# nikkolasg/playsnark

Measured on AMD Instinct MI355X. Metric: G1 scalar-muls/s (Pippenger MSM, 2^20 pts per GPU), higher is better.
Workload: dtype i32x14 (381-bit Fp, 28-bit unsaturated limbs, Montgomery); 1 GPU; BLS12-381 G1 MSM, 2^20 points per GPU, uniform 255-bit scalars; points_per_gpu=1048576, window_bits=20, windows=13, window_table=True, window_table_bytes=1744830464, slice=32, in_flight=4

## Files before the change

playsnark_amd/csrc/capi.hip:

```cpp
#include "../../include/playsnark_hip.h"

#include <hip/hip_runtime.h>

#include <algorithm>
#include <atomic>
#include <chrono>
#include <condition_variable>
#include <functional>
#include <mutex>
#include <cstdio>
#include <cstring>
#include <future>
#include <string>
#include <vector>

#include "msm.hpp"
#include "quotient.hpp"
#include "lagrange.hpp"

namespace ps {
#include "hostfield.inc"
}
using namespace ps;

// ... 970 lines not shown
                           (u32*)c->offs.p);
        hipLaunchKernelGGL(k_sort_big_scatter, dim3(big_grid), dim3(SORT_FINE), 0, st, (const unsigned short*)c->keys.p,
                           (const u32*)c->vals.p, (const u32*)coarse_off, (const u32*)tile_base, ncoarse, fb, (u32*)c->counts.p,
                           (u32*)c->sorted.p);
        }
    } else {
        HIP_TRY(hipMemsetAsync(c->counts.p, 0, 4 * G, st));
        {
            int bin_shift = 4;
            while ((pl.NB >> bin_shift) > (u32)DIGITS_BINS) bin_shift++;
            hipLaunchKernelGGL(k_digits_grouped, dgrid, dim3(DIGITS_THREADS), 2 * DIGITS_CHUNK * sizeof(u32), st, scalars_ptr(sc),
                               (u32)n, pl.c, pl.W, pl.NB, cadd, bin_shift, fold_neg, single, (u32*)c->counts.p, (u32*)c->keys.p,
                               (u32*)c->vals.p, (u32*)c->ranks.p);
        }
        PS_STAGE_MARK();
        hipLaunchKernelGGL(k_scan_blocks, dim3(scan_tiles), dim3(SCAN_BLOCK), 0, st, (const u32*)c->counts.p, (u32*)c->offs.p,
                           (u32*)c->bsum.p, (u64)G);
        hipLaunchKernelGGL(k_scan_top, dim3(1), dim3(1024), 0, st, (u32*)c->bsum.p, scan_tiles, (u32*)c->offs.p + G);
        hipLaunchKernelGGL(k_scan_add, dim3(scan_tiles), dim3(SCAN_BLOCK), 0, st, (u32*)c->offs.p, (const u32*)c->bsum.p, (u64)G);
        PS_STAGE_MARK();
        hipLaunchKernelGGL(k_scatter, dim3(nblocks(total)), dim3(256), 0, st, (const u32*)c->keys.p, (const u32*)c->vals.p,
                           (const u32*)c->ranks.p, (const u32*)c->offs.p, total, (u32*)c->sorted.p);
    }
    PS_STAGE_MARK();
    HIP_TRY(hipGetLastError());
    if (!pl.qtail) HIP_TRY(hipMemcpyAsync((char*)c->h_pinned + c->h_pinned_cap - 8, (u32*)c->offs.p + G, 4, hipMemcpyDeviceToHost, st));
    return PS_OK;
}

struct TableRef { const char* base; u64 stride; };
static bool table_ref(const ps_points* pts, size_t n, int wbits, int W, TableRef* out) {
    const Storage* st = pts->st;
    const size_t rb = table_row_bytes(pts->group);
    if (const void* t = st->table.load(std::memory_order_acquire)) {
        if (st->table_c == wbits && W <= st->table_W) {
            *out = TableRef{(const char*)t + pts->first * rb, (u64)st->table_stride};
            return true;
        }
    }
    if (const ViewTable* v = view_table_find(st, pts->first, n, wbits)) {
        const void* t = v->table.load(std::memory_order_acquire);
        if (t && W <= v->W) {
            *out = TableRef{(const char*)t, (u64)v->n};
            return true;
        }
    }
    return false;
}

template <class F>
static int msm_points_t(ps_ctx* c, ps_ctx* wc, const ps_points* pts, size_t n, const MsmPlan& pl, bool timed, int slot,
                        hipEvent_t wait_acc, hipEvent_t acc_done, bool inline_tail = false) {
    typedef typename KernelField<F>::type KF;
    constexpr unsigned LN = FieldTraits<KF>::LANES;
    const u64 total = (u64)pl.W * n;
    const u64 G = pl.G;
    const u32 nthreads_acc = (u32)((total + pl.M - 1) / pl.M);
    ReducePlan rp = reduce_plan(pl.NB);
    if (pl.qtail) {
        rp.small = false;
        rp.njobs = (u32)pl.c;
        rp.nblk = 1;
        rp.m = 0;
        rp.segs = ((1u << (pl.c - 1 - pl.rc_s)) + (1u << pl.rc_s) + 1) / 2;
    }
    const u32 nseg_total = rp.segs * (u32)pl.sets;
    const u32 per_role = rp.m * (u32)pl.sets, nres = rp.njobs * (u32)pl.sets;
    const bool tab = pl.table;
    const u32 pstride = tab ? (u32)table_row_bytes(pts->group) : (u32)sizeof(Affine<F>);
    TableRef tref{};
    if (tab && !table_ref(pts, n, pl.c, pl.W, &tref)) return fail(PS_ERR_ARG, "msm: internal: the plan names a window table the array does not carry");
    const char* src = tab ? tref.base : (const char*)points_ptr(pts);
    const u32 idx_mask = tab ? (1u << ENTRY_W_SHIFT) - 1u : 0x7fffffffu;
    const u64 w_stride = tab ? tref.stride : 0ull;
    int rc;
    if ((rc = wc->buckets.ensure(sizeof(Xyzz<F>) * G))) return rc;
    if ((rc = wc->parts.ensure(sizeof(Xyzz<F>) * 2 * (size_t)nthreads_acc))) return rc;
    if ((rc = wc->segs.ensure(sizeof(Xyzz<F>) * (2 * (size_t)nseg_total + 5 * (size_t)per_role + (size_t)nres * rp.nblk)))) return rc;
    if ((rc = wc->wins.ensure(sizeof(Xyzz<F>) * ((size_t)nres + (size_t)pl.sets) + 16))) return rc;
    const bool qfix = pl.shortsum && pl.lpb >= 1;
    const u32 qlpb = qfix ? std::min<u32>((u32)pl.lpb, 256 / QTraits<KF>::GL) : 0;
    const u64 heavy_slices = qfix ? std::min<u64>(HEAVY_SPAN, (u64)QFIX_HEAVY * qlpb - 1) : HEAVY_SPAN;
    const size_t max_heavy = (size_t)(total / (heavy_slices * (u64)pl.M)) + 2;
    if ((rc = wc->heavy.ensure(4 * (2 * max_heavy + 2)))) return rc;
    const u32 heavy_npb = 256 / QTraits<KF>::GL;
    const size_t max_jobs = (size_t)nthreads_acc / heavy_npb + max_heavy + 1;
    if ((rc = wc->hparts.ensure(sizeof(Xyzz<F>) * max_jobs))) return rc;
    if (sizeof(Xyzz<F>) * (pl.sets > 1 ? (size_t)pl.sets : (size_t)nres) + 16 > PS_PINNED_SLOT) return fail(PS_ERR_ARG, "too many windows");
    hipStream_t st = wc->stream;
    int evi = 4;
    if (wc->tail_used) HIP_TRY(hipStreamWaitEvent(st, wc->ev_tail_done, 0));
    if (storage_wait_ready(pts->st, st)) return fail(PS_ERR_HIP, "msm: event wait failed");
    if (wait_acc) HIP_TRY(hipStreamWaitEvent(st, wait_acc, 0));
    PS_STAGE_MARK();
    constexpr bool PF = LN == 1 || PS_G2_ACC_WAVES == 1;
    hipLaunchKernelGGL((k_accumulate<KF, PF>), dim3(nblocks((size_t)nthreads_acc * LN)), dim3(256), 0, st, src,
                       (const u32*)c->sorted.p, (const u32*)c->offs.p, (u32)G, pl.M, nthreads_acc, idx_mask, w_stride, pstride,
                       (Xyzz<F>*)wc->buckets.p, (Xyzz<F>*)wc->parts.p, (u32*)wc->heavy.p);
    if (acc_done) HIP_TRY(hipEventRecord(acc_done, st));
    PS_STAGE_MARK();
    HIP_TRY(hipEventRecord(wc->ev_acc_local, st));
    if (!inline_tail) {
        st = wc->tail;
        HIP_TRY(hipStreamWaitEvent(st, wc->ev_acc_local, 0));
    }
    if (pl.shortsum && pl.lpb >= 1) {
        const u32 lpb = qlpb;
        hipLaunchKernelGGL(k_qfixup<KF>, dim3(nblocks(G * (u64)lpb * QTraits<KF>::GL)), dim3(256), 0, st, (const u32*)c->offs.p, (u32)G, pl.M,
                           nthreads_acc, lpb, (const Xyzz<F>*)wc->parts.p, (Xyzz<F>*)wc->buckets.p, (u32*)wc->heavy.p, (u32*)wc->heavy.p + 1);
    } else
    hipLaunchKernelGGL(k_fixup<KF>, dim3(nblocks(G * LN)), dim3(256), 0, st, (const u32*)c->offs.p, (u32)G, pl.M, nthreads_acc,
                       (const Xyzz<F>*)wc->parts.p, (Xyzz<F>*)wc->buckets.p, (u32*)wc->heavy.p, (u32*)wc->heavy.p + 1);
    {
        const u32* hcount = (const u32*)wc->heavy.p;
        const u32* hlist = hcount + 1;
        u32* job_base = (u32*)wc->heavy.p + 1 + max_heavy;
        hipLaunchKernelGGL(k_heavy_jobs, dim3(1), dim3(256), 0, st, (const u32*)c->offs.p, (u32)G, pl.M, nthreads_acc, hcount, hlist, job_base, heavy_npb);
        hipLaunchKernelGGL(k_qfixup_heavy_part<KF>, dim3(1024), dim3(256), 0, st, (const u32*)c->offs.p, (u32)G, pl.M, nthreads_acc,
                           (const Xyzz<F>*)wc->parts.p,
                           hcount, hlist, (const u32*)job_base, (Xyzz<F>*)wc->hparts.p);
        hipLaunchKernelGGL(k_qfixup_heavy<KF>, dim3(256), dim3(256), 0, st, (const Xyzz<F>*)wc->hparts.p, (Xyzz<F>*)wc->buckets.p, hcount,
                           hlist, (const u32*)job_base);
    }
    PS_STAGE_MARK();
    {
        Xyzz<F>* accs = (Xyzz<F>*)wc->segs.p;
        Xyzz<F>* runs = accs + nseg_total;
        Xyzz<F>* lvl = runs + nseg_total;
        Xyzz<F>* pieces = lvl + 5 * (size_t)per_role;
        if (pl.qtail) {
            constexpr u32 QGL = QTraits<KF>::GL, QNP = 512 / QGL;
            const int cb = pl.c - 1, s = pl.rc_s;
            const u32 rows = 1u << (cb - s), cols = 1u << s;
            Xyzz<F>* R = accs;
            Xyzz<F>* C = accs + (size_t)pl.sets * rows;
            if (s > 0) {
                u32 np = std::min<u32>(QNP, std::max(rows, cols));
                while (np > 64 / QGL && (u64)np * QGL * (rows + cols) * (u32)pl.sets > 2048ull * 64) np >>= 1;
#if defined(PS_TAIL_TUNE)
                if (pl.busy) if (const char* e = getenv("PS_T_NP_BUSY")) np = std::max<u32>(64 / QGL, std::min<u32>(np, (u32)atoi(e)));
#endif
                hipLaunchKernelGGL(k_qreduce_rowcol<KF>, dim3((rows + cols) * (u32)pl.sets), dim3(np * QGL), np * QGL * sizeof(Fp), st,
                                   (const Xyzz<F>*)wc->buckets.p, cb, s, R, C, (const Xyzz<F>*)nullptr, (Xyzz<F>*)nullptr);
            }
            const u32 terms = std::max(rows, cols / 2);
            const u32 np = std::min<u32>(QNP, std::max<u32>(terms, 64 / QGL));
            hipLaunchKernelGGL(k_qreduce_bits<KF>, dim3(nres), dim3(np * QGL), np * QGL * sizeof(Fp), st,
                               s > 0 ? (const Xyzz<F>*)R : (const Xyzz<F>*)wc->buckets.p, (const Xyzz<F>*)C, cb, s, (Xyzz<F>*)wc->wins.p,
                               (const u32*)c->offs.p + G, (u32*)((Xyzz<F>*)wc->wins.p + (pl.sets > 1 ? nres + (size_t)pl.sets : (size_t)nres)),
                               (const Xyzz<F>*)nullptr);
        } else if (rp.small) {
            hipLaunchKernelGGL(k_reduce_small<KF>, dim3(nres), dim3(RED_SUM_LANES * LN), RED_SUM_LANES * sizeof(Xyzz<F>), st,
                               (const Xyzz<F>*)wc->buckets.p, pl.NB, rp.njobs, (Xyzz<F>*)wc->wins.p);
        } else {
            hipLaunchKernelGGL(k_reduce_l1<KF>, dim3(nblocks((size_t)nseg_total * LN)), dim3(256), 0, st, (const Xyzz<F>*)wc->buckets.p,
                               nseg_total, accs, runs);
            if (pl.hybrid && rp.segs >= 64) {
                constexpr u32 QGL = QTraits<KF>::GL, QNP = 256 / QGL;
                int cb2 = 0;
                while ((1u << cb2) < rp.segs) cb2++;
                const int s2 = (cb2 + 1) / 2;
                const u32 rows2 = 1u << (cb2 - s2), cols2 = 1u << s2;
                Xyzz<F>* R_run = lvl;
                Xyzz<F>* C_run = R_run + (size_t)pl.sets * rows2;
                Xyzz<F>* R_acc = C_run + (size_t)pl.sets * cols2;
                u32 np = std::min<u32>(QNP, std::max(rows2, cols2));
                while (np > 64 / QGL && (u64)np * QGL * (2 * rows2 + cols2) * (u32)pl.sets > 2048ull * 64) np >>= 1;
                hipLaunchKernelGGL(k_qreduce_rowcol<KF>, dim3((2 * rows2 + cols2) * (u32)pl.sets), dim3(np * QGL), np * QGL * sizeof(Fp), st,
                                   (const Xyzz<F>*)runs, cb2, s2, R_run, C_run, (const Xyzz<F>*)accs, R_acc);
                const u32 np2 = std::min<u32>(QNP, std::max<u32>(std::max(rows2, cols2 / 2), 64 / QGL));
                hipLaunchKernelGGL(k_qreduce_bits<KF>, dim3(nres), dim3(np2 * QGL), np2 * QGL * sizeof(Fp), st, (const Xyzz<F>*)R_run,
                                   (const Xyzz<F>*)C_run, cb2, s2, (Xyzz<F>*)wc->wins.p, (const u32*)nullptr, (u32*)nullptr, (const Xyzz<F>*)R_acc);
            } else {
            hipLaunchKernelGGL(k_reduce_pyr<KF>, dim3(nblocks(5 * (size_t)per_role * LN)), dim3(256), 0, st, (const Xyzz<F>*)accs,
                               (const Xyzz<F>*)runs, rp.segs, rp.m, (u32)pl.sets, lvl);
            hipLaunchKernelGGL(k_reduce_sum<KF>, dim3(nres * rp.nblk), dim3(RED_SUM_LANES * LN), RED_SUM_LANES * sizeof(Xyzz<F>), st,
                               (const Xyzz<F>*)lvl, rp.m, (u32)pl.sets, rp.njobs, rp.nblk, rp.nblk > 1 ? pieces : (Xyzz<F>*)wc->wins.p);
            if (rp.nblk > 1)
                hipLaunchKernelGGL(k_reduce_fin<KF>, dim3(nres), dim3(RED_SUM_LANES * LN), RED_SUM_LANES * sizeof(Xyzz<F>), st,
                                   (const Xyzz<F>*)pieces, rp.nblk, (Xyzz<F>*)wc->wins.p);
            }
        }
        if (pl.sets > 1)
            hipLaunchKernelGGL(k_reduce_weights<KF>, dim3((unsigned)pl.sets), dim3(RED_SUM_LANES * LN), RED_SUM_LANES * sizeof(Xyzz<F>), st,
                               (const Xyzz<F>*)wc->wins.p, rp.njobs, (rp.small && !pl.qtail) ? 1 : 0, pl.qtail ? 0 : RED_SEG_LOG,
                               (Xyzz<F>*)wc->wins.p + nres);
    }
    PS_STAGE_MARK();
    HIP_TRY(hipGetLastError());
    HIP_TRY(hipMemcpyAsync((char*)c->h_pinned + (size_t)slot * PS_PINNED_SLOT, (const Xyzz<F>*)wc->wins.p + (pl.sets > 1 ? nres : 0),
                           sizeof(Xyzz<F>) * (pl.sets > 1 ? (size_t)pl.sets : (size_t)nres) + (pl.qtail ? 4 : 0), hipMemcpyDeviceToHost, st));
    HIP_TRY(hipEventRecord(wc->ev_tail_done, st));
    wc->tail_used = true;
    return PS_OK;
}
#undef PS_STAGE_MARK

static bool table_usable(const ps_ctx* c, const ps_points* pts, size_t n, int max_bits) {
    const Storage* st = pts->st;
// ... 575 lines not shown
```

playsnark_amd/csrc/msm.hpp:

```cpp
#pragma once
#include "curve.hpp"

namespace ps {

#ifndef PS_TAIL_PRIO
#define PS_TAIL_PRIO 0
#endif
#if PS_TAIL_PRIO > 0
#define PS_TAIL_PRIO_HERE __builtin_amdgcn_s_setprio(PS_TAIL_PRIO)
#else
#define PS_TAIL_PRIO_HERE do { } while (0)
#endif

struct MsmPlan {
    int c;
    int W;
    u32 NB;
    u64 G;
    int M;
    int SEG;
    int sets;
    bool table;
    bool qtail;
    bool hybrid;
    bool shortsum;
    int lpb;
    int rc_s;
    bool busy;
};
constexpr int ENTRY_W_SHIFT = 26;

static inline MsmPlan msm_plan(size_t n, int max_bits, int forced_c) {
    MsmPlan best{};
    double best_cost = 1e300;
    for (int c = 4; c <= 20; c++) {
        if (forced_c ? c != forced_c : c > 16) continue;
        int W = max_bits / c + 1;
        double nb = (double)(1u << (c - 1));
        double cost = (double)n * W * 10.0 + W * nb * 42.0;
        if (cost < best_cost) {
            best_cost = cost;
            best.c = c;
            best.W = W;
        }
    }
    best.NB = 1u << (best.c - 1);
    best.sets = best.W;
    best.G = (u64)best.W * best.NB;
    best.M = 32;
    const u64 total = (u64)n * best.W;
    while (best.M < 1024 && total / (2 * (u64)best.M) >= (1u << 19)) best.M *= 2;
    while (best.M < 1024 && (u64)best.M * 5 * best.G < total) best.M *= 2;
    while (best.M > 8 && total / (u64)best.M < (1u << 17) && (u64)(best.M / 2) * 5 * best.G >= total) best.M /= 2;
    best.SEG = 8;
    return best;
}
static inline MsmPlan msm_plan_table(size_t n, int max_bits, int c) {
    MsmPlan pl{};
    pl.c = c;
    pl.W = max_bits / c + 1;
    pl.NB = 1u << (c - 1);
    pl.sets = 1;
    pl.table = true;
    pl.G = pl.NB;
    pl.M = 32;
    const u64 total = (u64)n * pl.W;
    while (pl.M < 1024 && total / (2 * (u64)pl.M) >= (1u << 19)) pl.M *= 2;
    while (pl.M < 1024 && (u64)pl.M * 5 * pl.G < total) pl.M *= 2;
    while (pl.M > 8 && total / (u64)pl.M < (1u << 17) && (u64)(pl.M / 2) * 5 * pl.G >= total) pl.M /= 2;
    pl.SEG = 8;
    return pl;
}

PS_INL u32 limb_sel8(const u32* k, int i) {
    u32 v = 0;
#pragma unroll
    for (int j = 0; j < 8; j++) v = (i == j) ? k[j] : v;
    return v;
}
constexpr int DIGITS_THREADS = 1024;
#ifndef PS_DIGITS_PER_THREAD
#define PS_DIGITS_PER_THREAD 8
#endif
constexpr int DIGITS_PER_THREAD = PS_DIGITS_PER_THREAD;
// ... 522 lines not shown
    __shared__ u32 hist[SORT_FINE];
    const u32 tid = threadIdx.x;
    for (u32 t = blockIdx.x;; t += gridDim.x) {
        u32 p, lo, hi;
        if (!sort_big_tile(t, tile_base, coarse_off, ncoarse, &p, &lo, &hi)) return;
        hist[tid] = 0;
        __syncthreads();
        u32 k[SORT_TILE_PER_THREAD];
#pragma unroll
        for (u32 j = 0; j < SORT_TILE_PER_THREAD; j++) {
            const u32 i = lo + j * SORT_FINE + tid;
            const bool act = i < hi;
            k[j] = act ? (u32)part_key[i] : 0xffffffffu;
            lds_count(hist, act ? k[j] : 0u, act);
        }
        __syncthreads();
        const u32 cnt = hist[tid];
        __syncthreads();
        hist[tid] = (tid < (1u << fb) && cnt) ? atomicAdd(&gcur[((size_t)p << fb) + tid], cnt) : 0u;
        __syncthreads();
#pragma unroll
        for (u32 j = 0; j < SORT_TILE_PER_THREAD; j++) {
            const bool act = k[j] != 0xffffffffu;
            const u32 pos = lds_rank(hist, act ? k[j] : 0u, act);
            if (act) sorted[pos] = part_val[lo + j * SORT_FINE + tid];
        }
        __syncthreads();
    }
}

template <class KF> struct FieldTraits { typedef KF Store; static constexpr int LANES = 1; };
template <> struct FieldTraits<Fp2s> { typedef Fp2 Store; static constexpr int LANES = 2; };
template <class S> struct KernelField { typedef S type; };
template <> struct KernelField<Fp2> { typedef Fp2s type; };

__device__ inline Fp ld_f(const Fp* p, const Fp*) { return *p; }
__device__ inline void st_f(Fp* p, const Fp& v) { *p = v; }
__device__ inline Fp2s ld_f(const Fp2* p, const Fp2s*) { return Fp2s{pair_lane() ? p->c1 : p->c0}; }
__device__ inline void st_f(Fp2* p, const Fp2s& v) { if (pair_lane()) p->c1 = v.v; else p->c0 = v.v; }

template <class KF>
__device__ inline Affine<KF> ld_affine(const Affine<typename FieldTraits<KF>::Store>* p) {
    Affine<KF> r;
    r.x = ld_f(&p->x, (const KF*)0);
    r.y = ld_f(&p->y, (const KF*)0);
    return r;
}
template <class KF>
__device__ inline Xyzz<KF> ld_xyzz(const Xyzz<typename FieldTraits<KF>::Store>* p) {
    Xyzz<KF> r;
    r.x = ld_f(&p->x, (const KF*)0);
    r.y = ld_f(&p->y, (const KF*)0);
    r.zz = ld_f(&p->zz, (const KF*)0);
    r.zzz = ld_f(&p->zzz, (const KF*)0);
    return r;
}
template <class KF>
__device__ inline void st_xyzz(Xyzz<typename FieldTraits<KF>::Store>* p, const Xyzz<KF>& v) {
    st_f(&p->x, v.x);
    st_f(&p->y, v.y);
    st_f(&p->zz, v.zz);
    st_f(&p->zzz, v.zzz);
}
template <class KF> __device__ inline u32 logical_tid() { return (blockIdx.x * blockDim.x + threadIdx.x) / FieldTraits<KF>::LANES; }
template <class KF> __device__ inline u32 logical_local() { return threadIdx.x / FieldTraits<KF>::LANES; }
template <class KF> __device__ inline u32 logical_block() { return blockDim.x / FieldTraits<KF>::LANES; }
template <class KF> __device__ inline bool pair_leader() { return FieldTraits<KF>::LANES == 1 || pair_lane() == 0; }

template <class KF>
__device__ inline void block_tree_sum(Xyzz<typename FieldTraits<KF>::Store>* sm, const Xyzz<KF>& mine) {
    const u32 lt = logical_local<KF>();
    st_xyzz<KF>(&sm[lt], mine);
    __syncthreads();
    for (u32 stride = logical_block<KF>() >> 1; stride > 0; stride >>= 1) {
        if (lt < stride) {
            Xyzz<KF> a = ld_xyzz<KF>(&sm[lt]), b = ld_xyzz<KF>(&sm[lt + stride]);
            xyzz_add_inl<KF>(a, b);
            st_xyzz<KF>(&sm[lt], a);
        }
        __syncthreads();
    }
}

__device__ inline int eff_slice(u32 E, u32 T, int M) {
#if defined(PS_NO_EFF_SLICE)
    return M;
#endif
    const u64 m = (4ull * E + T - 1) / (T ? T : 1u);
    const u64 lo = M < 4 ? (u64)M : 4ull;
    return m >= (u64)M ? M : (int)(m < lo ? lo : m);
}

template <class F>
PS_INL bool affine_is_identity(const Affine<F>& p) { return fp_all_zero(p.x) && fp_all_zero(p.y); }

template <class KF>
__device__ inline void flush_run(const Xyzz<KF>& acc, u32 g, u32 rs, u32 re, u32 slice_start, u32 t,
                                 const u32* __restrict__ offs, Xyzz<typename FieldTraits<KF>::Store>* __restrict__ buckets,
                                 Xyzz<typename FieldTraits<KF>::Store>* __restrict__ parts) {
    bool whole = (rs == offs[g]) && (re == offs[g + 1]);
    if (whole) st_xyzz<KF>(&buckets[g], acc);
    else if (rs == slice_start) st_xyzz<KF>(&parts[2 * (size_t)t], acc);
    else st_xyzz<KF>(&parts[2 * (size_t)t + 1], acc);
}

template <class KF>
__device__ inline Affine<KF> ld_entry_point(const char* __restrict__ points, u32 e, u32 idx_mask, u64 w_stride, u32 pstride) {
    const size_t row = (size_t)(e & idx_mask) + (size_t)((e >> ENTRY_W_SHIFT) & 31u) * w_stride;
    return ld_affine<KF>(reinterpret_cast<const Affine<typename FieldTraits<KF>::Store>*>(points + row * pstride));
}

__device__ inline void next_bucket(const u32* __restrict__ offs, u32 G, u32 p, u32& g, u32& bend) {
    g++;
    bend = offs[g + 1];
    if (bend > p) return;
    u32 lo = g + 1, hi = G;
    while (hi - lo > 1) {
        const u32 mid = (lo + hi) >> 1;
        if (offs[mid] <= p) lo = mid; else hi = mid;
    }
    g = lo;
    bend = offs[g + 1];
}

#ifndef PS_G2_ACC_WAVES
#define PS_G2_ACC_WAVES 2
#endif
#define PS_ACC_WAVES(KF) (FieldTraits<KF>::LANES == 2 ? PS_G2_ACC_WAVES : 2)
template <class KF, bool PREFETCH>
__global__ void __launch_bounds__(256, PS_ACC_WAVES(KF)) k_accumulate(const char* __restrict__ points,
                                                       const u32* __restrict__ sorted, const u32* __restrict__ offs,
                                                       u32 G, int Mplan, u32 T, u32 idx_mask, u64 w_stride, u32 pstride,
                                                       Xyzz<typename FieldTraits<KF>::Store>* __restrict__ buckets,
                                                       Xyzz<typename FieldTraits<KF>::Store>* __restrict__ parts,
                                                       u32* __restrict__ heavy_count) {
    const u32 E = offs[G];
    const int M = eff_slice(E, T, Mplan);
    const u32 t = logical_tid<KF>();
    if (blockIdx.x == 0 && threadIdx.x == 0) *heavy_count = 0;
    const u64 start64 = (u64)t * (u64)M;
    if (start64 >= E) return;
    const u32 start = (u32)start64;
    const u32 end = (E - start < (u32)M) ? E : start + (u32)M;
    u32 lo = 0, hi = G;
    while (hi - lo > 1) {
        u32 mid = (lo + hi) >> 1;
        if (offs[mid] <= start) lo = mid; else hi = mid;
    }
    u32 g = lo;
    u32 bend = offs[g + 1];
    u32 run_start = start;
    Xyzz<KF> acc = xyzz_identity<KF>();
    if (PREFETCH) {
        u32 e = sorted[start];
        u32 e1 = start + 1 < end ? sorted[start + 1] : e;
        Affine<KF> pt = ld_entry_point<KF>(points, e, idx_mask, w_stride, pstride);
        for (u32 p = start; p < end; p++) {
            Affine<KF> nxt = pt;
            u32 e2 = e1;
            if (p + 1 < end) nxt = ld_entry_point<KF>(points, e1, idx_mask, w_stride, pstride);
            if (p + 2 < end) e2 = sorted[p + 2];
            if (p >= bend) {
                flush_run<KF>(acc, g, run_start, p, start, t, offs, buckets, parts);
                acc = xyzz_identity<KF>();
                run_start = p;
                next_bucket(offs, G, p, g, bend);
            }
            if (!affine_is_identity<KF>(pt)) {
                if (e >> 31) pt.y = f_neg(pt.y);
                xyzz_madd_inl<KF>(acc, pt.x, pt.y);
            }
            pt = nxt; e = e1; e1 = e2;
        }
    } else {
        for (u32 p = start; p < end; p++) {
            if (p >= bend) {
                flush_run<KF>(acc, g, run_start, p, start, t, offs, buckets, parts);
                acc = xyzz_identity<KF>();
                run_start = p;
                next_bucket(offs, G, p, g, bend);
            }
            const u32 e = sorted[p];
            Affine<KF> pt = ld_entry_point<KF>(points, e, idx_mask, w_stride, pstride);
            if (!affine_is_identity<KF>(pt)) {
                if (e >> 31) pt.y = f_neg(pt.y);
                xyzz_madd_inl<KF>(acc, pt.x, pt.y);
            }
        }
    }
    flush_run<KF>(acc, g, run_start, end, start, t, offs, buckets, parts);
}

constexpr u32 HEAVY_SPAN = 8;

#ifndef PS_TAIL_WAVES
#define PS_TAIL_WAVES 2
#endif

template <class KF>
__global__ void __launch_bounds__(256, PS_TAIL_WAVES) k_fixup(const u32* __restrict__ offs, u32 G, int Mplan, u32 T,
                                                  const Xyzz<typename FieldTraits<KF>::Store>* __restrict__ parts,
                                                  Xyzz<typename FieldTraits<KF>::Store>* __restrict__ buckets,
                                                  u32* __restrict__ heavy_count, u32* __restrict__ heavy_list) {
    PS_TAIL_PRIO_HERE;
    u32 g = logical_tid<KF>();
    if (g >= G) return;
    const int M = eff_slice(offs[G], T, Mplan);
    u32 lo = offs[g], hi = offs[g + 1];
    if (lo == hi) {
        st_xyzz<KF>(&buckets[g], xyzz_identity<KF>());
        return;
    }
    u32 t0 = lo / (u32)M, t1 = (hi - 1) / (u32)M;
    if (t0 == t1) return;
    if (t1 - t0 >= HEAVY_SPAN) {
        if (pair_leader<KF>()) heavy_list[atomicAdd(heavy_count, 1u)] = g;
        return;
    }
    Xyzz<KF> acc = xyzz_identity<KF>();
    for (u32 t = t0; t <= t1; t++) {
        u32 slice_start = t * (u32)M;
        u32 rs = lo > slice_start ? lo : slice_start;
        Xyzz<KF> part = ld_xyzz<KF>(&parts[2 * (size_t)t + (rs == slice_start ? 0 : 1)]);
        xyzz_add_inl<KF>(acc, part);
    }
    st_xyzz<KF>(&buckets[g], acc);
}

constexpr u32 HEAVY_CHUNK = 1024;
__host__ __device__ inline u32 heavy_chunk_of(u32 span, u32 npb) {
    u32 s = 1;
    while ((u64)s * s * npb * npb < span) s++;
    return npb * s;
}

__global__ void __launch_bounds__(256) k_heavy_jobs(const u32* __restrict__ offs, u32 G, int Mplan, u32 T, const u32* __restrict__ heavy_count,
                                                    const u32* __restrict__ heavy_list, u32* __restrict__ job_base, u32 npb) {
    PS_TAIL_PRIO_HERE;
    const int M = eff_slice(offs[G], T, Mplan);
    __shared__ u32 wsum[4];
    const u32 nheavy = *heavy_count;
    const u32 tid = threadIdx.x;
    u32 running = 0;
    for (u32 base = 0; base < nheavy; base += 256) {
        const u32 h = base + tid;
        u32 cnt = 0;
        if (h < nheavy) {
            const u32 g = heavy_list[h];
            const u32 t0 = offs[g] / (u32)M, t1 = (offs[g + 1] - 1) / (u32)M;
            const u32 chunk = npb ? heavy_chunk_of(t1 - t0 + 1, npb) : HEAVY_CHUNK;
            cnt = (t1 - t0 + chunk) / chunk;
        }
        u32 inc = wave_incl_scan(cnt);
        if ((tid & 63) == 63) wsum[tid >> 6] = inc;
        __syncthreads();
        u32 before = 0, tile = 0;
        for (u32 q = 0; q < 4; q++) {
            if (q < (tid >> 6)) before += wsum[q];
            tile += wsum[q];
        }
        if (h < nheavy) job_base[h] = running + before + inc - cnt;
        running += tile;
        __syncthreads();
    }
    if (tid == 0) job_base[nheavy] = running;
}


#ifndef PS_RED_SEG_LOG
#define PS_RED_SEG_LOG 3
#endif
constexpr int RED_SEG_LOG = PS_RED_SEG_LOG;
constexpr int RED_SEG = 1 << RED_SEG_LOG;
constexpr int RED_DIRECT_JOBS = 4;
constexpr u32 RED_SUM_LANES = 64;
#ifndef PS_RED_SUM_TERMS
#define PS_RED_SUM_TERMS 512
#endif
constexpr u32 RED_SUM_TERMS = PS_RED_SUM_TERMS;

struct ReducePlan {
    u32 segs;
    u32 m;
    int kb;
    u32 njobs;
    u32 nblk;
    bool small;
};
constexpr u32 RED_SMALL_NB = 1024;
static inline ReducePlan reduce_plan(u32 NB) {
    ReducePlan r;
    r.small = NB <= RED_SMALL_NB;
    if (r.small) {
        r.segs = r.m = 0;
        r.kb = 0;
        r.njobs = 1;
        while ((1u << (r.njobs - 1)) < NB) r.njobs++;
        r.nblk = 1;
        return r;
    }
    r.segs = NB >> RED_SEG_LOG;
    r.m = r.segs >= 8 ? r.segs / 8 : 1;
    r.kb = 0;
    while ((1u << r.kb) < r.m) r.kb++;
    r.njobs = RED_DIRECT_JOBS + (u32)r.kb;
    r.nblk = r.m / RED_SUM_TERMS;
    if (r.nblk < 1) r.nblk = 1;
    if (r.nblk > RED_SUM_LANES) r.nblk = RED_SUM_LANES;
// ... 469 lines not shown
```

playsnark_amd/csrc/qtail.hpp:

```cpp
#pragma once

namespace ps {

template <class KF> struct QTraits {
    static constexpr int S = FieldTraits<KF>::LANES;
    static constexpr int GL = 4 * S;
};
PS_INL Fp& fp_of(Fp& a) { return a; }
PS_INL const Fp& fp_of(const Fp& a) { return a; }
PS_INL Fp& fp_of(Fp2s& a) { return a.v; }
PS_INL const Fp& fp_of(const Fp2s& a) { return a.v; }

#if defined(__HIP_DEVICE_COMPILE__)
__device__ inline i32 lane_read(i32 v, int src_lane) { return __builtin_amdgcn_ds_bpermute(src_lane << 2, v); }
#else
PS_HD inline i32 lane_read(i32 v, int) { return v; }
#endif

template <class KF> __device__ inline int q_coord() { return (int)((threadIdx.x / QTraits<KF>::S) & 3u); }

template <class KF>
__device__ inline KF q_get(const KF& v, int src) {
    constexpr int S = QTraits<KF>::S;
    const int lane = (int)(threadIdx.x & 63u);
// ... 80 lines not shown
        fp_of(ob).l[i] = odd ? fp_of(b).l[i] : fp_of(d).l[i];
    }
    const KF e = f_mul_ilp(oa, ob);
    const KF PP = q_bcast<0>(e), Pd = q_bcast<1>(d);
#pragma unroll
    for (int i = 0; i < FP_L; i++) {
        fp_of(oa).l[i] = j == 0 ? fp_of(m).l[i] : j == 1 ? fp_of(e).l[i] : fp_of(Pd).l[i];
        fp_of(ob).l[i] = j == 0 ? fp_of(e).l[i] : fp_of(PP).l[i];
    }
    const KF f = f_mul_ilp(oa, ob);
    const KF QQ = q_bcast<0>(f);
    const KF x3 = f_norm(f_sub(f_sub(f_sub(e, f), QQ), QQ));
    const KF x3q = f_sub(x3, QQ);
    KF oc, od;
#pragma unroll
    for (int i = 0; i < FP_L; i++) {
        fp_of(oa).l[i] = j == 2 ? fp_of(d).l[i] : fp_of(e).l[i];
        fp_of(ob).l[i] = j == 2 ? fp_of(x3q).l[i] : fp_of(f).l[i];
        fp_of(oc).l[i] = j == 2 ? fp_of(m).l[i] : 0;
        fp_of(od).l[i] = j == 2 ? fp_of(f).l[i] : 0;
    }
    const KF g = f_mul2sub_ilp(oa, ob, oc, od);
    const KF X3 = q_bcast<2>(x3);
    a = q_select<KF>(X3, f, f_norm(g), g, j);
}

template <class KF>
__device__ inline void q_block_tree(Fp* sm, KF& mine, u32 pt, u32 grp) {
    constexpr u32 GL = QTraits<KF>::GL;
    const u32 sub = pt & (grp - 1);
    for (u32 stride = grp >> 1; stride > 0; stride >>= 1) {
        if (sub >= stride && sub < 2 * stride) sm[threadIdx.x] = fp_of(mine);
        __syncthreads();
        if (sub < stride) {
            KF o;
            fp_of(o) = sm[threadIdx.x + stride * GL];
            q_add<KF>(mine, o);
        }
    }
}

constexpr u32 QFIX_HEAVY = 16;
template <class KF>
__global__ void __launch_bounds__(256) k_qfixup(const u32* __restrict__ offs, u32 G, int Mplan, u32 T, u32 LPB,
                                                const Xyzz<typename FieldTraits<KF>::Store>* __restrict__ parts,
                                                Xyzz<typename FieldTraits<KF>::Store>* __restrict__ buckets,
                                                u32* __restrict__ heavy_count, u32* __restrict__ heavy_list) {
    PS_TAIL_PRIO_HERE;
    constexpr u32 GL = QTraits<KF>::GL;
    __shared__ Fp sm[256];
    const int M = eff_slice(offs[G], T, Mplan);
    const u32 pt = threadIdx.x / GL;
    const u64 gp = (u64)blockIdx.x * (256 / GL) + pt;
    const u32 g = (u32)(gp / LPB), sub = (u32)(gp % LPB);
    const bool valid = g < G;
    KF acc = f_zero((const KF*)0);
    bool store = false;
    if (valid) {
        const u32 lo = offs[g], hi = offs[g + 1];
        if (lo == hi) {
            store = true;
        } else {
            const u32 t0 = lo / (u32)M, t1 = (hi - 1) / (u32)M;
            if (t0 != t1) {
                if (t1 - t0 >= QFIX_HEAVY * LPB) {
                    if (sub == 0 && (threadIdx.x & (GL - 1)) == 0) heavy_list[atomicAdd(heavy_count, 1u)] = g;
                } else {
                    store = true;
                    for (u32 t = t0 + sub; t <= t1; t += LPB) {
                        const u32 slice_start = t * (u32)M;
                        const u32 rs = lo > slice_start ? lo : slice_start;
                        const KF p = q_load<KF>(&parts[2 * (size_t)t + (rs == slice_start ? 0 : 1)]);
                        q_add<KF>(acc, p);
                    }
                }
            }
        }
    }
    q_block_tree<KF>(sm, acc, pt, LPB);
    if (store && sub == 0) q_store<KF>(&buckets[g], acc);
}

template <class KF>
__device__ inline u32 q_tree_size(u32 count) {
    constexpr u32 NPB = 256 / QTraits<KF>::GL;
    u32 g = 1;
    while (g < count && g < NPB) g <<= 1;
    return g;
}
template <class KF>
__global__ void __launch_bounds__(256) k_qfixup_heavy_part(const u32* __restrict__ offs, u32 G, int Mplan, u32 T,
                                                            const Xyzz<typename FieldTraits<KF>::Store>* __restrict__ parts,
                                                            const u32* __restrict__ heavy_count, const u32* __restrict__ heavy_list,
                                                            const u32* __restrict__ job_base,
                                                            Xyzz<typename FieldTraits<KF>::Store>* __restrict__ hparts) {
    PS_TAIL_PRIO_HERE;
    constexpr u32 GL = QTraits<KF>::GL, NPB = 256 / GL;
    __shared__ Fp sm[256];
    const u32 nheavy = *heavy_count;
    if (nheavy == 0) return;
    const int M = eff_slice(offs[G], T, Mplan);
    const u32 njobs = job_base[nheavy];
    const u32 pt = threadIdx.x / GL;
    for (u32 j = blockIdx.x; j < njobs; j += gridDim.x) {
        u32 lo_h = 0, hi_h = nheavy;
        while (hi_h - lo_h > 1) {
            const u32 mid = (lo_h + hi_h) >> 1;
            if (job_base[mid] <= j) lo_h = mid; else hi_h = mid;
        }
        const u32 g = heavy_list[lo_h];
        const u32 lo = offs[g], hi = offs[g + 1];
        const u32 t0 = lo / (u32)M, t1 = (hi - 1) / (u32)M;
        const u32 chunk = heavy_chunk_of(t1 - t0 + 1, NPB);
        const u32 ts = t0 + (j - job_base[lo_h]) * chunk;
        const u32 te = (t1 - ts >= chunk) ? ts + chunk - 1 : t1;
        KF acc = f_zero((const KF*)0);
        for (u32 t = ts + pt; t <= te; t += NPB) {
            const u32 slice_start = t * (u32)M;
            const u32 rs = lo > slice_start ? lo : slice_start;
            const KF p = q_load<KF>(&parts[2 * (size_t)t + (rs == slice_start ? 0 : 1)]);
            q_add<KF>(acc, p);
        }
        q_block_tree<KF>(sm, acc, pt, q_tree_size<KF>(te - ts + 1));
        if (pt == 0) q_store<KF>(&hparts[j], acc);
        __syncthreads();
    }
}
template <class KF>
__global__ void __launch_bounds__(256) k_qfixup_heavy(const Xyzz<typename FieldTraits<KF>::Store>* __restrict__ hparts,
                                                       Xyzz<typename FieldTraits<KF>::Store>* __restrict__ buckets,
                                                       const u32* __restrict__ heavy_count, const u32* __restrict__ heavy_list,
                                                       const u32* __restrict__ job_base) {
    PS_TAIL_PRIO_HERE;
    constexpr u32 GL = QTraits<KF>::GL, NPB = 256 / GL;
    __shared__ Fp sm[256];
    const u32 nheavy = *heavy_count;
    const u32 pt = threadIdx.x / GL;
    for (u32 h = blockIdx.x; h < nheavy; h += gridDim.x) {
        const u32 j0 = job_base[h], j1 = job_base[h + 1];
        KF acc = f_zero((const KF*)0);
        for (u32 j = j0 + pt; j < j1; j += NPB) { const KF p = q_load<KF>(&hparts[j]); q_add<KF>(acc, p); }
        q_block_tree<KF>(sm, acc, pt, q_tree_size<KF>(j1 - j0));
        if (pt == 0) q_store<KF>(&buckets[heavy_list[h]], acc);
        __syncthreads();
    }
}

template <class KF>
__global__ void __launch_bounds__(512) k_qreduce_rowcol(const Xyzz<typename FieldTraits<KF>::Store>* __restrict__ buckets, int cb, int s,
                                                         Xyzz<typename FieldTraits<KF>::Store>* __restrict__ R,
                                                         Xyzz<typename FieldTraits<KF>::Store>* __restrict__ C,
                                                         const Xyzz<typename FieldTraits<KF>::Store>* __restrict__ extra,
                                                         Xyzz<typename FieldTraits<KF>::Store>* __restrict__ R2) {
    PS_TAIL_PRIO_HERE;
    constexpr u32 GL = QTraits<KF>::GL;
    extern __shared__ __align__(16) unsigned char smem_raw[];
    Fp* sm = reinterpret_cast<Fp*>(smem_raw);
    const u32 rows = 1u << (cb - s), cols = 1u << s, jobs = rows + cols + (extra ? rows : 0u);
    const u32 set = blockIdx.x / jobs, job = blockIdx.x % jobs;
    const bool second = job >= rows + cols;
    const Xyzz<typename FieldTraits<KF>::Store>* B = (second ? extra : buckets) + ((size_t)set << cb);
    const u32 pt = threadIdx.x / GL, NP = blockDim.x / GL;
    KF acc = f_zero((const KF*)0);
    if (job < rows || second) {
        const u32 row = second ? job - rows - cols : job;
        for (u32 i = pt; i < cols; i += NP) { const KF p = q_load<KF>(&B[(size_t)row * cols + i]); q_add<KF>(acc, p); }
// ... 44 lines not shown
```

Baseline: 418.7 million G1 scalar-muls/s.

## Split bucket fixup into classify, pair, and chain kernels

When the short-sum path is off, the single per-bucket fixup kernel is replaced by three kernels. A classify pass marks empty, chain and heavy buckets. A per-slice-boundary kernel merges two-part buckets, and a quad-lane kernel reduces chain buckets listed by the classify pass. The goal is to remove divergence and load imbalance in the per-bucket fixup, at the cost of extra launches, atomics and a binary search per boundary. The heavy-list layout gains a second counter slot.

```diff
diff --git a/playsnark_amd/csrc/capi.hip b/playsnark_amd/csrc/capi.hip
--- a/playsnark_amd/csrc/capi.hip
+++ b/playsnark_amd/csrc/capi.hip
@@ -1076,7 +1076,13 @@
     const u32 qlpb = qfix ? std::min<u32>((u32)pl.lpb, 256 / QTraits<KF>::GL) : 0;
     const u64 heavy_slices = qfix ? std::min<u64>(HEAVY_SPAN, (u64)QFIX_HEAVY * qlpb - 1) : HEAVY_SPAN;
     const size_t max_heavy = (size_t)(total / (heavy_slices * (u64)pl.M)) + 2;
-    if ((rc = wc->heavy.ensure(4 * (2 * max_heavy + 2)))) return rc;
+#if defined(PS_FIXUP_ONE_KERNEL)
+    const bool split_fixup = false;
+#else
+    const bool split_fixup = !pl.shortsum;
+#endif
+    const size_t max_chain = split_fixup ? (size_t)nthreads_acc / 2 + 2 : 0;
+    if ((rc = wc->heavy.ensure(4 * (2 * max_heavy + 3 + max_chain)))) return rc;
     const u32 heavy_npb = 256 / QTraits<KF>::GL;
     const size_t max_jobs = (size_t)nthreads_acc / heavy_npb + max_heavy + 1;
     if ((rc = wc->hparts.ensure(sizeof(Xyzz<F>) * max_jobs))) return rc;
@@ -1101,14 +1107,26 @@
     if (pl.shortsum && pl.lpb >= 1) {
         const u32 lpb = qlpb;
         hipLaunchKernelGGL(k_qfixup<KF>, dim3(nblocks(G * (u64)lpb * QTraits<KF>::GL)), dim3(256), 0, st, (const u32*)c->offs.p, (u32)G, pl.M,
-                           nthreads_acc, lpb, (const Xyzz<F>*)wc->parts.p, (Xyzz<F>*)wc->buckets.p, (u32*)wc->heavy.p, (u32*)wc->heavy.p + 1);
+                           nthreads_acc, lpb, (const Xyzz<F>*)wc->parts.p, (Xyzz<F>*)wc->buckets.p, (u32*)wc->heavy.p, (u32*)wc->heavy.p + 2);
+    } else if (split_fixup) {
+        u32* ccount = (u32*)wc->heavy.p + 1;
+        u32* clist = (u32*)wc->heavy.p + 2 + 2 * max_heavy + 1;
+        hipLaunchKernelGGL(k_fixup_classify<KF>, dim3(nblocks(G * LN)), dim3(256), 0, st, (const u32*)c->offs.p, (u32)G, pl.M, nthreads_acc,
+                           (Xyzz<F>*)wc->buckets.p, (u32*)wc->heavy.p, (u32*)wc->heavy.p + 2, ccount, clist);
+        if (nthreads_acc > 1)
+            hipLaunchKernelGGL(k_fixup_pair<KF>, dim3(nblocks((size_t)(nthreads_acc - 1) * LN)), dim3(256), 0, st, (const u32*)c->offs.p, (u32)G,
+                               pl.M, nthreads_acc, (const Xyzz<F>*)wc->parts.p, (Xyzz<F>*)wc->buckets.p);
+        constexpr u32 chain_npb = 256 / QTraits<KF>::GL;
+        hipLaunchKernelGGL(k_qfixup_chain<KF>, dim3((unsigned)std::min<size_t>((max_chain + chain_npb - 1) / chain_npb, 512)), dim3(256), 0, st,
+                           (const u32*)c->offs.p, (u32)G, pl.M, nthreads_acc, (const Xyzz<F>*)wc->parts.p, (Xyzz<F>*)wc->buckets.p,
+                           (const u32*)ccount, (const u32*)clist);
     } else
     hipLaunchKernelGGL(k_fixup<KF>, dim3(nblocks(G * LN)), dim3(256), 0, st, (const u32*)c->offs.p, (u32)G, pl.M, nthreads_acc,
-                       (const Xyzz<F>*)wc->parts.p, (Xyzz<F>*)wc->buckets.p, (u32*)wc->heavy.p, (u32*)wc->heavy.p + 1);
+                       (const Xyzz<F>*)wc->parts.p, (Xyzz<F>*)wc->buckets.p, (u32*)wc->heavy.p, (u32*)wc->heavy.p + 2);
     {
         const u32* hcount = (const u32*)wc->heavy.p;
-        const u32* hlist = hcount + 1;
-        u32* job_base = (u32*)wc->heavy.p + 1 + max_heavy;
+        const u32* hlist = hcount + 2;
+        u32* job_base = (u32*)wc->heavy.p + 2 + max_heavy;
         hipLaunchKernelGGL(k_heavy_jobs, dim3(1), dim3(256), 0, st, (const u32*)c->offs.p, (u32)G, pl.M, nthreads_acc, hcount, hlist, job_base, heavy_npb);
         hipLaunchKernelGGL(k_qfixup_heavy_part<KF>, dim3(1024), dim3(256), 0, st, (const u32*)c->offs.p, (u32)G, pl.M, nthreads_acc,
                            (const Xyzz<F>*)wc->parts.p,
diff --git a/playsnark_amd/csrc/fixup_class.hpp b/playsnark_amd/csrc/fixup_class.hpp
--- /dev/null
+++ b/playsnark_amd/csrc/fixup_class.hpp
@@ -0,0 +1,47 @@
+#pragma once
+#include "field.hpp"
+
+namespace ps {
+
+PS_HD inline int eff_slice(u32 E, u32 T, int M) {
+#if defined(PS_NO_EFF_SLICE)
+    return M;
+#endif
+    const u64 m = (4ull * E + T - 1) / (T ? T : 1u);
+    const u64 lo = M < 4 ? (u64)M : 4ull;
+    return m >= (u64)M ? M : (int)(m < lo ? lo : m);
+}
+
+constexpr u32 HEAVY_SPAN = 8;
+
+enum BucketClass : int {
+    BUCKET_EMPTY = 0,
+    BUCKET_WHOLE = 1,
+    BUCKET_PAIR = 2,
+    BUCKET_CHAIN = 3,
+    BUCKET_HEAVY = 4
+};
+PS_HD inline int bucket_class(u32 lo, u32 hi, u32 M, u32 heavy_span) {
+    if (lo == hi) return BUCKET_EMPTY;
+    const u32 span = (hi - 1) / M - lo / M;
+    return span == 0 ? BUCKET_WHOLE : span >= heavy_span ? BUCKET_HEAVY : span == 1 ? BUCKET_PAIR : BUCKET_CHAIN;
+}
+
+PS_HD inline size_t part_slot(u32 lo, u32 t, u32 M) { return 2 * (size_t)t + (lo > t * M ? 1 : 0); }
+
+PS_HD inline bool pair_boundary_bucket(const u32* __restrict__ offs, u32 G, u32 E, u32 t, u32 M, u32 heavy_span, u32& g) {
+    const u64 pos64 = (u64)t * M;
+    if (pos64 >= E) return false;
+    const u32 pos = (u32)pos64;
+    u32 lo = 0, hi = G;
+    while (hi - lo > 1) {
+        const u32 mid = (lo + hi) >> 1;
+        if (offs[mid] <= pos) lo = mid; else hi = mid;
+    }
+    g = lo;
+    const u32 b0 = offs[lo], b1 = offs[lo + 1];
+    if (b0 == pos) return false;
+    return bucket_class(b0, b1, M, heavy_span) == BUCKET_PAIR;
+}
+
+}
diff --git a/playsnark_amd/csrc/msm.hpp b/playsnark_amd/csrc/msm.hpp
--- a/playsnark_amd/csrc/msm.hpp
+++ b/playsnark_amd/csrc/msm.hpp
@@ -1,5 +1,6 @@
 #pragma once
 #include "curve.hpp"
+#include "fixup_class.hpp"
 
 namespace ps {
 
@@ -688,14 +689,6 @@
     }
 }
 
-__device__ inline int eff_slice(u32 E, u32 T, int M) {
-#if defined(PS_NO_EFF_SLICE)
-    return M;
-#endif
-    const u64 m = (4ull * E + T - 1) / (T ? T : 1u);
-    const u64 lo = M < 4 ? (u64)M : 4ull;
-    return m >= (u64)M ? M : (int)(m < lo ? lo : m);
-}
 
 template <class F>
 PS_INL bool affine_is_identity(const Affine<F>& p) { return fp_all_zero(p.x) && fp_all_zero(p.y); }
@@ -743,7 +736,7 @@
     const u32 E = offs[G];
     const int M = eff_slice(E, T, Mplan);
     const u32 t = logical_tid<KF>();
-    if (blockIdx.x == 0 && threadIdx.x == 0) *heavy_count = 0;
+    if (blockIdx.x == 0 && threadIdx.x == 0) heavy_count[0] = heavy_count[1] = 0;
     const u64 start64 = (u64)t * (u64)M;
     if (start64 >= E) return;
     const u32 start = (u32)start64;
@@ -797,7 +790,6 @@
     flush_run<KF>(acc, g, run_start, end, start, t, offs, buckets, parts);
 }
 
-constexpr u32 HEAVY_SPAN = 8;
 
 #ifndef PS_TAIL_WAVES
 #define PS_TAIL_WAVES 2
@@ -830,6 +822,42 @@
         Xyzz<KF> part = ld_xyzz<KF>(&parts[2 * (size_t)t + (rs == slice_start ? 0 : 1)]);
         xyzz_add_inl<KF>(acc, part);
     }
+    st_xyzz<KF>(&buckets[g], acc);
+}
+
+template <class KF>
+__global__ void __launch_bounds__(256) k_fixup_classify(const u32* __restrict__ offs, u32 G, int Mplan, u32 T,
+                                                        Xyzz<typename FieldTraits<KF>::Store>* __restrict__ buckets,
+                                                        u32* __restrict__ heavy_count, u32* __restrict__ heavy_list,
+                                                        u32* __restrict__ chain_count, u32* __restrict__ chain_list) {
+    PS_TAIL_PRIO_HERE;
+    const u32 g = logical_tid<KF>();
+    if (g >= G) return;
+    const int M = eff_slice(offs[G], T, Mplan);
+    const int cls = bucket_class(offs[g], offs[g + 1], (u32)M, HEAVY_SPAN);
+    if (cls == BUCKET_EMPTY) {
+        st_xyzz<KF>(&buckets[g], xyzz_identity<KF>());
+    } else if (cls == BUCKET_CHAIN) {
+        if (pair_leader<KF>()) chain_list[atomicAdd(chain_count, 1u)] = g;
+    } else if (cls == BUCKET_HEAVY) {
+        if (pair_leader<KF>()) heavy_list[atomicAdd(heavy_count, 1u)] = g;
+    }
+}
+
+template <class KF>
+__global__ void __launch_bounds__(256, PS_TAIL_WAVES) k_fixup_pair(const u32* __restrict__ offs, u32 G, int Mplan, u32 T,
+                                                       const Xyzz<typename FieldTraits<KF>::Store>* __restrict__ parts,
+                                                       Xyzz<typename FieldTraits<KF>::Store>* __restrict__ buckets) {
+    PS_TAIL_PRIO_HERE;
+    const u32 t = logical_tid<KF>() + 1;
+    if (t >= T) return;
+    const u32 E = offs[G];
+    const int M = eff_slice(E, T, Mplan);
+    u32 g;
+    if (!pair_boundary_bucket(offs, G, E, t, (u32)M, HEAVY_SPAN, g)) return;
+    Xyzz<KF> acc = ld_xyzz<KF>(&parts[part_slot(offs[g], t - 1, (u32)M)]);
+    const Xyzz<KF> right = ld_xyzz<KF>(&parts[2 * (size_t)t]);
+    xyzz_add_inl<KF>(acc, right);
     st_xyzz<KF>(&buckets[g], acc);
 }
 
diff --git a/playsnark_amd/csrc/qtail.hpp b/playsnark_amd/csrc/qtail.hpp
--- a/playsnark_amd/csrc/qtail.hpp
+++ b/playsnark_amd/csrc/qtail.hpp
@@ -186,6 +186,28 @@
 }
 
 template <class KF>
+__global__ void __launch_bounds__(256) k_qfixup_chain(const u32* __restrict__ offs, u32 G, int Mplan, u32 T,
+                                                      const Xyzz<typename FieldTraits<KF>::Store>* __restrict__ parts,
+                                                      Xyzz<typename FieldTraits<KF>::Store>* __restrict__ buckets,
+                                                      const u32* __restrict__ chain_count, const u32* __restrict__ chain_list) {
+    PS_TAIL_PRIO_HERE;
+    constexpr u32 GL = QTraits<KF>::GL, NPB = 256 / GL;
+    const u32 nchain = *chain_count;
+    const int M = eff_slice(offs[G], T, Mplan);
+    for (u32 h = blockIdx.x * NPB + threadIdx.x / GL; h < nchain; h += gridDim.x * NPB) {
+        const u32 g = chain_list[h];
+        const u32 lo = offs[g], hi = offs[g + 1];
+        const u32 t0 = lo / (u32)M, t1 = (hi - 1) / (u32)M;
+        KF acc = q_load<KF>(&parts[part_slot(lo, t0, (u32)M)]);
+        for (u32 t = t0 + 1; t <= t1; t++) {
+            const KF p = q_load<KF>(&parts[2 * (size_t)t]);
+            q_add<KF>(acc, p);
+        }
+        q_store<KF>(&buckets[g], acc);
+    }
+}
+
+template <class KF>
 __device__ inline u32 q_tree_size(u32 count) {
     constexpr u32 NPB = 256 / QTraits<KF>::GL;
     u32 g = 1;
```

Result: faster. 425.1 million G1 scalar-muls/s (median of 6 runs) (+1.5%).
